# wangsibovictor/fora

Measured on AMD Instinct MI355X. Metric: SSPPR queries/sec at eps=0.5, higher is better.
Workload: dtype u64 fixed-point 2^-62 (f64 at the boundary)

## Files before the change

### fora_amd/csrc/fora_diag.h

```cpp
#pragma once
#include <hip/hip_runtime.h>
#include <stdint.h>

#if defined(FORA_STAMPS) || defined(FORA_STAMPS_SMALL) || defined(FORA_STAMPS_LEVELS) || defined(FORA_PROBE_STORE) || defined(FORA_PROBE_STORE2) || \
    defined(FORA_PROBE_GATHER) || defined(FORA_PROBE_BIN_LOAD) || defined(FORA_PROBE_BIN_RANK) || defined(FORA_PROBE_BIN_STORE) ||              \
    defined(FORA_PROBE_BIN_SYNC) || defined(FORA_PROBE_BIN_LDS) || defined(FORA_PROBE_ACC_LOAD) || defined(FORA_PROBE_ACC_ATOM) ||               \
    defined(FORA_PROBE_ACC_SWEEP) || defined(FORA_DG_FAKE_STEP0) || defined(FORA_DG_FAKE_ALL)
#define FORA_DIAG_BUILD 1
#else
#define FORA_DIAG_BUILD 0
#endif

#ifdef FORA_STAMPS
#define STAMP_DECL long long st_t_ = clock64(); unsigned long long st_a_[8] = {0, 0, 0, 0, 0, 0, 0, 0}; (void)st_a_;
#define STAMP(slot) do { const long long n_ = clock64(); st_a_[(slot) & 7] += (unsigned long long)(n_ - st_t_); st_t_ = n_; } while (0)
#define STAMP_FLUSH(base) do { if (threadIdx.x == 0) for (int i_ = 0; i_ < 8; i_++) if (st_a_[i_]) atomicAdd(&d.stamps[(base) + i_], st_a_[i_]); } while (0)
#define TSTAMP_DECL long long ts_t_ = clock64(); unsigned long long ts_a_[10] = {0, 0, 0, 0, 0, 0, 0, 0, 0, 0}; bool ts_on_ = true; (void)ts_on_;
#ifdef FORA_STAMPS_SMALL
#define TSTAMP(k) do { const long long n_ = clock64(); if (ts_on_) ts_a_[k] += (unsigned long long)(n_ - ts_t_); ts_t_ = n_; } while (0)
#define TSTAMP_GATE(F) do { ts_on_ = (F) <= (uint32_t)(FORA_STAMPS_SMALL) && (F) > 0; if (ts_on_) ts_a_[4]++; } while (0)
#else
#define TSTAMP(k) do { const long long n_ = clock64(); ts_a_[k] += (unsigned long long)(n_ - ts_t_); ts_t_ = n_; } while (0)
#define TSTAMP_GATE(F) do {} while (0)
#endif
// ... 20 lines not shown
namespace fora {
namespace diag {

__device__ __forceinline__ void keep(uint32_t x) { asm volatile("" ::"v"(x)); }
__device__ __forceinline__ void keep(uint64_t x) { asm volatile("" ::"v"(x)); }
__device__ __forceinline__ void keep(const uint4 &x) { asm volatile("" ::"v"(x.x), "v"(x.y), "v"(x.z), "v"(x.w)); }
__device__ __forceinline__ unsigned long long opaque_zero() { unsigned long long z = 0; asm volatile("" : "+v"(z)); return z; }

#if defined(FORA_PROBE_STORE) || defined(FORA_PROBE_STORE2)
constexpr size_t TEAM_MSG_PROBE_WORDS = (size_t)80000000 + (1u << 18);
#else
constexpr size_t TEAM_MSG_PROBE_WORDS = 0;
#endif

template <int EPT>
__device__ __forceinline__ void team_emit_probe(const uint32_t (&word)[EPT], const uint32_t (&dst)[EPT], const uint32_t (&slot)[EPT], uint32_t *mout, uint32_t empty) {
#ifdef FORA_PROBE_STORE2
    {
        const uint32_t base = (uint32_t)__builtin_amdgcn_readfirstlane((int)slot[0]) & ~63u, lane_ = threadIdx.x & 63u;
#pragma unroll
        for (int k = 0; k < EPT; k++)
            mout[(size_t)80000000 + base + k * 4096 + (FORA_PROBE_STORE2 == 1 ? lane_ : (lane_ >> 4) * 1024 + (lane_ & 15u) + 5)] = word[k];
    }
#endif
#ifdef FORA_PROBE_STORE
#pragma unroll
    for (int k = 0; k < EPT; k++)
        if (dst[k] != empty) mout[(size_t)(FORA_PROBE_STORE) + slot[k]] = word[k];
#endif
    (void)word; (void)dst; (void)slot; (void)mout; (void)empty;
}
__device__ __forceinline__ uint64_t team_gather_probe(const uint64_t *tb, uint32_t entry, bool have) {
#ifdef FORA_PROBE_GATHER
    const uint64_t xa = __hip_atomic_load((const unsigned long long *)&tb[have ? (entry ^ 8u) : 0u], __ATOMIC_RELAXED, __HIP_MEMORY_SCOPE_AGENT);
    return xa >> 63;
#else
    (void)tb; (void)entry; (void)have;
    return 0;
#endif
}

__device__ __forceinline__ uint32_t dg_from(uint32_t cur, uint32_t t) {
#if defined(FORA_DG_FAKE_ALL)
    (void)t; return cur & 1023u;
#elif defined(FORA_DG_FAKE_STEP0)
    return t == 0 ? (cur & 1023u) : cur;
#else
    (void)t; return cur;
#endif
}

__device__ __forceinline__ uint4 bin_load_probe(const int32_t *colsrc, const int32_t *col4, const int32_t *col_hub4, const int32_t *col, int64_t quad) {
#if defined(FORA_PROBE_BIN_LOAD) && FORA_PROBE_BIN_LOAD == 2
// ... 98 lines not shown
```

### fora_amd/csrc/fora_hip.hip

```cpp
#include "fora_kernels.h"
#include "fora_team.h"
#include "fora_bwd.h"
#include "../../include/fora_hip.h"

#include <algorithm>
#include <cmath>
#include <cstdio>
#include <cstdlib>
#include <cstring>
#include <string>
#include <vector>

using namespace fora;

struct fora_ctx;
static int build_hub_copy(fora_ctx *c, const int64_t *row_ptr, const int32_t *col);
static int build_quad_copies(fora_ctx *c);
namespace {

struct EvPair {
    hipEvent_t a, b;
    int kind;
};

// ... 29 lines not shown
    int64_t team_hubs = 1024;
    int64_t tail_hubs = 1;
    int64_t team_log = -1;
    int64_t slot_major = -1;
    int64_t acc_group = 0;
    int64_t team_abort_level = 0;
    int64_t team_timeout_ms = 500;
    int64_t team_coop = 0;
    int64_t topk_bk_div = 16;
    int64_t quads = 1;
    int64_t pipeline = 0;
    int64_t profile = 1;
    int64_t grid = 2048;
    int64_t bwd_lds_cap = BWD_CAP_DEFAULT;
    int64_t bwd_chunk = 0;
};
static const struct { const char *name; int64_t Tunables::*field; bool layout; } OPTIONS[] = {
    {"direct", &Tunables::direct, true}, {"force_wide", &Tunables::force_wide, true}, {"pass_bins", &Tunables::pass_bins, true},
    {"no_split", &Tunables::no_split, true}, {"no_compact", &Tunables::no_compact, false}, {"walk_dg", &Tunables::walk_dg, false}, {"dg_hubs", &Tunables::dg_hubs, false}, {"hubs", &Tunables::hubs, true}, {"hubs_wide", &Tunables::hubs_wide, true}, {"hub_min", &Tunables::hub_min, false}, {"bkcap", &Tunables::bkcap, true},
    {"ovcap", &Tunables::ovcap, true}, {"tiny", &Tunables::tiny, false}, {"xb", &Tunables::xb, false}, {"ax", &Tunables::ax, false},
    {"wx", &Tunables::wx, false}, {"tail", &Tunables::tail, false}, {"tail_always", &Tunables::tail_always, false},
    {"select_compact", &Tunables::select_compact, false}, {"pipeline", &Tunables::pipeline, false}, {"team", &Tunables::team, true}, {"team_size", &Tunables::team_size, true}, {"team_tail", &Tunables::team_tail, false}, {"team_xcd", &Tunables::team_xcd, false}, {"team_max", &Tunables::team_max, true}, {"team_hubs", &Tunables::team_hubs, true}, {"team_log", &Tunables::team_log, false}, {"topk_bk_div", &Tunables::topk_bk_div, true}, {"quads", &Tunables::quads, false}, {"team_timeout_ms", &Tunables::team_timeout_ms, false}, {"team_abort_level", &Tunables::team_abort_level, false}, {"acc_group", &Tunables::acc_group, false}, {"slot_major", &Tunables::slot_major, false}, {"team_coop", &Tunables::team_coop, false}, {"tail_hubs", &Tunables::tail_hubs, false}, {"rounds", &Tunables::rounds, false}, {"defer", &Tunables::defer, true}, {"defer_min", &Tunables::defer_min, false}, {"round_div", &Tunables::round_div, false},
    {"profile", &Tunables::profile, false}, {"grid", &Tunables::grid, false},
    {"bwd_lds_cap", &Tunables::bwd_lds_cap, false}, {"bwd_chunk", &Tunables::bwd_chunk, false},
};
static bool schedule_option(const char *name) {
    return !strcmp(name, "rounds") || !strcmp(name, "round_div") || !strcmp(name, "defer") || !strcmp(name, "defer_min");
}
static Tunables tunables_from_env() {
    Tunables t;
    for (const auto &o : OPTIONS) {
        if (schedule_option(o.name)) continue;
        std::string env = "FORA_HIP_";
        for (const char *p = o.name; *p; p++) env += (char)toupper((unsigned char)*p);
        if (const char *e = getenv(env.c_str())) if (*e) t.*(o.field) = atoll(e);
    }
    return t;
}

struct fora_ctx {
    int device = 0;
    Tunables opt_;
    hipStream_t stream = nullptr;
    std::string err;
    hipDeviceProp_t prop{};

    int32_t n = 0;
// ... 18 lines not shown
    uint64_t *d_hubsum = nullptr;
    uint32_t *d_dg_perm = nullptr, *d_dg_inv = nullptr, *d_dg_colp = nullptr, *d_dg_rec = nullptr, *d_dg_invb = nullptr;
    uint8_t *d_dg_T = nullptr;
    WalkDG dg{};
    uint32_t *d_colt = nullptr, *d_team_off = nullptr, *d_team_n2l = nullptr, *d_team_l2n = nullptr;
    uint32_t *d_team_hubtgt = nullptr;
    uint32_t team_H = 0, team_hubs_opt = 0;
    uint16_t *d_team_rlog_id = nullptr; uint64_t *d_team_rlog_val = nullptr; uint32_t team_rlog_cap = 0;
    uint64_t *d_team_rowl = nullptr, *d_team_rsvl = nullptr;
    uint16_t *d_team_deg16 = nullptr;
    uint32_t *d_team_rowq = nullptr;
    uint32_t team_T = 0, team_R = 0, team_force = 0;
    bool team_checked = false, team_wanted = false;
    double dangling_frac = 0;
    uint64_t team_cap = 0;
    uint32_t *d_team_msg = nullptr;
    uint64_t *d_team_inct = nullptr;
    unsigned long long *d_team_cnt = nullptr;
    uint32_t *d_team_ctl = nullptr;
    uint32_t team_n = 0;
    bool team_dirty = false;
    bool hub_for_team = false;
    bool team_timeout_seen = false;
    int team_suspend = 0;
    uint64_t team_fallbacks = 0;
    int team_fit = -1;
    bool team_coop_ok = false;
    bool team_coop_failed = false;

    bool have_params = false;
    double alpha = 0.2, epsilon = 0.5, rmax_scale = 1.0, rmax = 0, omega = 0;
// ... 381 lines not shown
               c->wit_cap >= pe.wits && c->bk_cap == pe.bk_cap && c->sub == pe.sub;
    };
    {
        int need = c->batch_req > 0 ? c->batch_req : std::min(want_slots > 0 ? want_slots : 1024, 1024);
        if (c->batch_req == 0 && c->B > 0 && c->B_memcap > 0) need = std::min(need, c->B_memcap);
        if (keepable(need)) { const WsPlan pe = plan_workspace(c, omega_hint, c->B); return ensure_row_split(c, pe.nbins, pe.pbins); }
    }
    int B = c->batch_req > 0 ? c->batch_req : 0;
    if (B == 0) {
        free_workspace(c);
        size_t fr = 0, tot = 0;
        HIPCHK(c, hipMemGetInfo(&fr, &tot));
        uint64_t budget = (uint64_t)(fr * (c->opt_.pipeline == 1 ? 0.4 : 0.75));
        if (c->team_T) {
            const uint64_t T = c->team_T, nt = std::max<uint64_t>(1, (uint64_t)c->prop.multiProcessorCount * TEAM_WGS_PER_CU / T);
            const uint64_t team_bytes = nt * (2 * c->team_cap * 4 + 3 * T * (c->team_R + 64 + c->team_H) * 8 + T * (10ull << 17) + 2 * T * T * 8);
            budget -= std::min<uint64_t>(budget / 2, team_bytes);
        }
        B = (int)std::min<uint64_t>(1024, std::max<uint64_t>(1, budget / p.per_slot));
    }
    B = std::max(1, B);
    const int memcap = B;
    if (want_slots > 0 && c->batch_req == 0) B = std::min(B, std::max(want_slots, 1));
    p = plan_workspace(c, omega_hint, B);
    const uint64_t scratch = (uint64_t)B * p.scratch;
    free_workspace(c);
    const uint64_t slab = (uint64_t)B * n;
    HIPCHK(c, hipMalloc(&c->d_residue, slab * 8));
    HIPCHK(c, hipMalloc(&c->d_ppr, slab * 8));
    if (p.binned) {
        HIPCHK(c, hipMalloc(&c->d_fl[0], slab * 4));
// ... 12 lines not shown
        HIPCHK(c, hipMalloc(&c->d_bk_count, (size_t)B * p.pbins * p.sub * 4));
        HIPCHK(c, hipHostMalloc(&c->h_flc, (size_t)FLC_RING * B * 4 * CSTRIDE));
        c->dbm_words = (uint32_t)((uint64_t)p.nbins << (bin_shift(c) - 6));
        HIPCHK(c, hipMalloc(&c->d_dbm, 2 * (size_t)B * c->dbm_words * 8));
        HIPCHK(c, hipMalloc(&c->d_dflag, 2 * (size_t)B * p.nbins * 4));
        if (c->opt_.defer > 0) HIPCHK(c, hipMalloc(&c->d_dl, 2 * slab * 4));
        if (c->hubs && c->hub_shift == bin_shift(c)) HIPCHK(c, hipMalloc(&c->d_hubsum, (size_t)B * p.sub * c->hubs * 8));
        if (c->team_T) {
            const uint32_t T = c->team_T;
            uint32_t nteams = std::max<uint32_t>(1, (uint32_t)c->prop.multiProcessorCount * TEAM_WGS_PER_CU / T);
            if (c->opt_.team_max > 0) nteams = std::min<uint32_t>(nteams, (uint32_t)c->opt_.team_max);
            size_t fr = 0, tot = 0;
            HIPCHK(c, hipMemGetInfo(&fr, &tot));
            c->team_rlog_cap = 1u << 17;
            auto per_team_bytes = [&](uint32_t logcap) {
                return 2 * c->team_cap * 4 + 3 * (uint64_t)T * (c->team_R + 64 + c->team_H) * 8 + (uint64_t)T * logcap * 10 + 2 * (uint64_t)T * T * 8;
            };
            while (c->team_rlog_cap > 1024 && per_team_bytes(c->team_rlog_cap) > fr / 4) c->team_rlog_cap /= 2;
            const uint64_t per_team = per_team_bytes(c->team_rlog_cap);
            nteams = (uint32_t)std::max<uint64_t>(1, std::min<uint64_t>(nteams, (uint64_t)(fr / 2) / std::max<uint64_t>(1, per_team)));
            HIPCHK(c, hipMalloc(&c->d_team_msg, (size_t)nteams * 2 * c->team_cap * 4 + 64 + diag::TEAM_MSG_PROBE_WORDS * 4));
            HIPCHK(c, hipMalloc(&c->d_team_inct, (size_t)nteams * 2 * T * (c->team_R + 64 + c->team_H) * 8));
            HIPCHK(c, hipMalloc(&c->d_team_rsvl, (size_t)nteams * T * c->team_R * 8));
            HIPCHK(c, hipMemset(c->d_team_rsvl, 0, (size_t)nteams * T * c->team_R * 8));
            HIPCHK(c, hipMalloc(&c->d_team_rlog_id, (size_t)nteams * T * c->team_rlog_cap * 2));
            HIPCHK(c, hipMalloc(&c->d_team_rlog_val, (size_t)nteams * T * c->team_rlog_cap * 8));
            HIPCHK(c, hipMalloc(&c->d_team_cnt, (size_t)nteams * 2 * T * T * 8));
            HIPCHK(c, hipMalloc(&c->d_team_ctl, (64 + (size_t)nteams * 5 * 16 * 2 + (size_t)nteams * ((size_t)B + 2)) * 4));
            c->team_n = nteams;
            if (int rf = team_fits(c)) return rf;
        }
    } else {
        HIPCHK(c, hipMalloc(&c->d_wl[0], slab * 8));
        HIPCHK(c, hipMalloc(&c->d_wl[1], slab * 8));
    }
    HIPCHK(c, hipMalloc(&c->d_scratch, scratch));
// ... 321 lines not shown
    a.residue = d.residue; a.ppr = d.ppr; a.fl0 = d.fl[0]; a.fl_count0 = d.fl_count[0]; a.inc_tab0 = d.inc_tab[0];
    a.segq_cap = d.segq_cap; a.qs = d.qs; a.err = d.err; a.afix = d.afix; a.t1 = d.t1;
    a.T = T; a.R = c->team_R; a.nteams = nteams;
    a.colt = c->d_colt; a.rowq = c->d_team_rowq; a.n2l = c->d_team_n2l; a.l2n = c->d_team_l2n; a.deg16 = c->d_team_deg16; a.rowl = c->d_team_rowl; a.rsvl = c->d_team_rsvl; a.rlog_id = c->d_team_rlog_id; a.rlog_val = c->d_team_rlog_val; a.rlog_cap = c->opt_.team_log == 0 ? 0u : c->opt_.team_log > 0 ? std::min<uint32_t>((uint32_t)c->opt_.team_log, c->team_rlog_cap) : c->team_rlog_cap; a.H = c->team_H; a.hubtgt = c->d_team_hubtgt; a.off = c->d_team_off; a.msg = c->d_team_msg; a.inct = c->d_team_inct; a.cntw = c->d_team_cnt;
    a.ctl = c->d_team_ctl;
    a.sync = (unsigned long long *)(c->d_team_ctl + 64);
    a.slot_seq = c->d_team_ctl + 64 + (size_t)nteams * 5 * 16 * 2;
    const int64_t tail_auto = 4096;
    a.tail_max = (uint32_t)std::min<int64_t>(std::max<int64_t>(c->opt_.team_tail < 0 ? tail_auto : c->opt_.team_tail, 0), 0x7FFFFFFF);
    if (c->opt_.tail == 0) a.tail_max = 0;
    a.tail_always = c->opt_.tail_always == 1 ? 1u : 0u;
    const uint32_t grid = nteams * T;
    a.xcd = (c->opt_.team_xcd >= 1 && grid % 8 == 0 && (grid / 8) % T == 0) ? (uint32_t)c->opt_.team_xcd : 0u;
    a.stamps = c->d_stamps;
    a.abort_level = (uint32_t)std::min<int64_t>(std::max<int64_t>(c->opt_.team_abort_level, 0), 1 << 20);
    a.timeout_ticks = (uint64_t)std::min<int64_t>(std::max<int64_t>(c->opt_.team_timeout_ms, 0), 60000) * 100000ull;
    const size_t lds = ((size_t)a.R + 1 + a.H) * 8;
    if (c->team_dirty) { HIPCHK(c, hipMemsetAsync(c->d_team_rsvl, 0, (size_t)nteams * T * c->team_R * 8, c->stream)); c->team_dirty = false; }
    HIPCHK(c, hipMemsetAsync(c->d_team_ctl, 0, (64 + (size_t)nteams * 5 * 16 * 2) * 4, c->stream));
    HIPCHK(c, hipMemsetAsync(c->d_team_cnt, 0, (size_t)nteams * 2 * T * T * 8, c->stream));
    HIPCHK(c, hipMemsetAsync(a.slot_seq, 0xFF, (size_t)nteams * ((size_t)d.nq + 2) * 4, c->stream));
    int h = ev_begin(c, 10);
    bool launched = false;
    if (c->team_coop_ok && !c->team_coop_failed) {
        void *args[] = {(void *)&a};
        const hipError_t le = hipLaunchCooperativeKernel((const void *)k_push_team, dim3(grid), dim3(TEAM_THREADS), args, (unsigned)lds, c->stream);
        if (le == hipSuccess) launched = true;
        else { (void)hipGetLastError(); c->team_coop_failed = true; }
    }
    if (!launched) hipLaunchKernelGGL(k_push_team, dim3(grid), dim3(TEAM_THREADS), lds, c->stream, a);
// ... 829 lines not shown
int fora_hip_get_batch(fora_ctx *c) { return c ? c->B : FORA_E_ARG; }

int fora_hip_set_option(fora_ctx *c, const char *name, int64_t value) {
    if (!c || !name) return FORA_E_ARG;
    if (!strcmp(name, "reset")) {
        (void)hipSetDevice(c->device);
        free_workspace(c);
        if (c->twin) free_workspace(c->twin);
        c->opt_ = tunables_from_env();
        c->team_suspend = 0;
        c->profiling = c->opt_.profile != 0;
        c->grid_blocks = c->opt_.grid > 0 ? (int)c->opt_.grid : 2048;
        if (c->twin) { c->twin->opt_ = c->opt_; c->twin->grid_blocks = c->grid_blocks; }
        return FORA_OK;
    }
    if (!TEST_PATHS && schedule_option(name) && value != (strcmp(name, "rounds") ? (strcmp(name, "round_div") ? 0 : 4) : 1))
        return fail(c, FORA_E_ARG, std::string("option ") + name + ": the schedule experiments are not compiled into this library (build with -DFORA_TEST_PATHS=1: libfora_hip_test.so)");
    for (const auto &o : OPTIONS)
        if (!strcmp(name, o.name)) {
            if (c->opt_.*(o.field) == value) return FORA_OK;
            c->opt_.*(o.field) = value;
            if (o.layout) { (void)hipSetDevice(c->device); free_workspace(c); if (c->twin) free_workspace(c->twin); }
            if (!strcmp(name, "profile")) c->profiling = value != 0;
            if (!strcmp(name, "grid")) { c->grid_blocks = value > 0 ? (int)value : 2048; if (c->twin) c->twin->grid_blocks = c->grid_blocks; }
            return FORA_OK;
        }
    return fail(c, FORA_E_ARG, std::string("unknown option ") + name);
}

int fora_hip_get_option(fora_ctx *c, const char *name, int64_t *value) {
    if (!name || !value) return FORA_E_ARG;
// ... 1139 lines not shown
```

### fora_amd/csrc/fora_team.h

```cpp
#pragma once
#include "fora_kernels.h"

namespace fora {

constexpr int TEAM_MAX = 32;
constexpr int TEAM_LBITS = 15;
#ifndef FORA_TEAM_THREADS
#define FORA_TEAM_THREADS 1024
#endif
constexpr int TEAM_THREADS = FORA_TEAM_THREADS;
#ifndef FORA_TEAM_WGS_PER_CU
#define FORA_TEAM_WGS_PER_CU (FORA_TEAM_THREADS == 1024 ? 1 : 2)
#endif
constexpr int TEAM_WGS_PER_CU = FORA_TEAM_WGS_PER_CU;
constexpr int TEAM_NW = TEAM_THREADS / 64;
constexpr uint32_t TEAM_R_CAP = TEAM_WGS_PER_CU == 1 ? 15296 : 7680;
constexpr int TEAM_NIT = (TEAM_R_CAP + TEAM_THREADS - 1) / TEAM_THREADS;
#ifndef FORA_TEAM_EPT
#define FORA_TEAM_EPT 4
#endif
#ifndef FORA_TEAM_CU
#define FORA_TEAM_CU 4
#endif
#ifndef FORA_TEAM_MPL
#define FORA_TEAM_MPL 2
#endif
#ifndef FORA_TEAM_DRAW
#define FORA_TEAM_DRAW 4
#endif
constexpr int TEAM_EPT = FORA_TEAM_EPT;
constexpr int TEAM_CHUNK = 64 * TEAM_EPT;
constexpr uint32_t TEAM_LMASK = (1u << TEAM_LBITS) - 1u;
constexpr uint32_t TEAM_EMPTY = 0xFFFFFFFFu;
constexpr uint32_t ERR_TEAM_TIMEOUT = 16, ERR_TEAM_CAP = 32;

struct TeamDev {
    int32_t n, nq;
    const uint64_t *rowinfo;
    const int64_t *row_ptr;
    const uint32_t *deg;
    const int32_t *src;
    uint64_t *residue, *ppr;
    uint32_t *fl0, *fl_count0;
    uint64_t *inc_tab0;
    uint64_t segq_cap;
    QState *qs;
    uint32_t *err;
    uint64_t afix, t1;
    uint32_t T, R, nteams;
    const uint32_t *colt;
    const uint32_t *rowq;
    const uint32_t *n2l;
    const uint32_t *l2n;
    const uint16_t *deg16;
    const uint64_t *rowl;
    uint64_t *rsvl;
    uint16_t *rlog_id;
    uint64_t *rlog_val;
    uint32_t rlog_cap;
    uint32_t H;
    const uint32_t *hubtgt;
    const uint32_t *off;
    uint32_t *msg;
    uint64_t *inct;
    unsigned long long *cntw;
    unsigned long long *sync;
    uint32_t *slot_seq;
    uint32_t *ctl;
    uint32_t tail_max;
    uint32_t tail_always;
    uint32_t xcd;
    unsigned long long *stamps;
    uint64_t timeout_ticks;
    uint32_t abort_level;
};

typedef const __attribute__((address_space(4))) TeamDev *TeamArgs;
__device__ __forceinline__ TeamArgs team_args() {
    TeamArgs p = (TeamArgs)__builtin_amdgcn_kernarg_segment_ptr();
    asm volatile("" : "+s"(p));
    return p;
}

__device__ __forceinline__ uint32_t rank_below(unsigned long long mk) {
    return __builtin_amdgcn_mbcnt_hi((uint32_t)(mk >> 32), __builtin_amdgcn_mbcnt_lo((uint32_t)mk, 0u));
}
__device__ __forceinline__ int fresh(int x) { asm volatile("" : "+v"(x)); return x; }
__device__ __forceinline__ uint32_t fresh_s(uint32_t x) { asm volatile("" : "+s"(x)); return x; }

// ... 26 lines not shown


#ifndef FORA_TEAM_HEAVY
#define FORA_TEAM_HEAVY 1024
#endif
constexpr uint32_t TEAM_HEAVY = FORA_TEAM_HEAVY;
#ifndef FORA_TEAM_NHEAVY
#define FORA_TEAM_NHEAVY 128
#endif
#ifndef FORA_TEAM_MAXGROUPS
#define FORA_TEAM_MAXGROUPS 256
#endif
constexpr int TEAM_NHEAVY = FORA_TEAM_NHEAVY;
constexpr int TEAM_MAXGROUPS = FORA_TEAM_MAXGROUPS;

__device__ __forceinline__ void team_emit(const uint32_t (&word)[TEAM_EPT], const uint32_t (&dst)[TEAM_EPT], uint32_t *s_fill, uint32_t *mout) {
    uint32_t slot[TEAM_EPT];
#pragma unroll
    for (int k = 0; k < TEAM_EPT; k++) {
        slot[k] = 0;
        if (dst[k] != TEAM_EMPTY) slot[k] = atomicAdd(&s_fill[dst[k]], 1u);
    }
#pragma unroll
    for (int k = 0; k < TEAM_EPT; k++)
        if (dst[k] != TEAM_EMPTY) mout[slot[k]] = word[k];
    diag::team_emit_probe(word, dst, slot, mout, TEAM_EMPTY);
}

__global__ void __launch_bounds__(TEAM_THREADS, TEAM_THREADS * TEAM_WGS_PER_CU / 256) k_push_team(const TeamDev kernarg_only) {
    extern __shared__ uint64_t res[];
    __shared__ uint16_t w_list[TEAM_NW][128];
// ... 107 lines not shown
            src_spare = src_word == TEAM_EMPTY;
            src_local = src_spare ? R : (src_word & TEAM_LMASK);
        }
        uint64_t acc_res = 0, acc_pops = 0, acc_relax = 0;
        uint32_t peak = 0, nlev = 0;
        uint32_t logbase = 0;
        bool final_round = false;
        if (fresh(tid0) == 0) s_rsvovf = 0;

        TSTAMP_LEVEL_DECL
        for (uint32_t L = 0;; L++) {
            const int tid = fresh(tid0), lane = tid & 63, wid = __builtin_amdgcn_readfirstlane(tid >> 6);
            if (L > 0) {
                const TeamArgs a = team_args();
                const uint32_t par = (g - 1) & 1u;
                const uint32_t *min_ = a->msg + ((uint64_t)team * 2 + par) * cap_total;
                const uint64_t *tin = a->inct + ((uint64_t)team * 2 + par) * T * tstride;
                const uint32_t tagp = g & 0xFFFFFFu;
                const unsigned long long *cwin = a->cntw + ((uint64_t)team * 2 + par) * T * T + (uint64_t)me * T;
                const unsigned long long full = T >= 64 ? ~0ull : (1ull << T) - 1ull;
                unsigned long long donemask = 0;
                uint32_t fsum = 0, spins = 0;
                uint64_t w_t0 = 0;
                while (donemask != full) {
                unsigned long long wv = 0;
                if ((uint32_t)lane < T) wv = __hip_atomic_load(&cwin[lane], __ATOMIC_RELAXED, __HIP_MEMORY_SCOPE_AGENT);
                const unsigned long long ready = __ballot((uint32_t)lane < T && (uint32_t)(wv >> 40) == tagp) & ~donemask;
                if (!ready) {
                    TSTAMP_SLEEP(8, 2, 40);
                    if ((++spins & 255u) == 0) {
                        const TeamArgs ar = team_args();
// ... 3 lines not shown
                        bool stop = __hip_atomic_load(&ctl[32], __ATOMIC_RELAXED, __HIP_MEMORY_SCOPE_AGENT) != 0;
                        if (!stop && now - w_t0 > ar->timeout_ticks) {
                            __hip_atomic_store(&ctl[32], 1u, __ATOMIC_RELAXED, __HIP_MEMORY_SCOPE_AGENT);
                            if (lane == 0) atomicOr(ar->err, ERR_TEAM_TIMEOUT);
                            stop = true;
                        }
                        if (stop) { if (lane == 0) s_abort = 1u; break; }
                    }
                    continue;
                }
                if (!same_xcd) { __builtin_amdgcn_fence(__ATOMIC_ACQUIRE, "agent"); asm volatile("s_waitcnt vmcnt(0)" ::: "memory"); }
                donemask |= ready;
                const bool mine = (ready >> lane) & 1ull;
                const uint32_t c = mine ? (uint32_t)wv & 0xFFFFFFu : 0u;
                fsum += mine ? (uint32_t)(wv >> 24) & 0xFFFFu : 0u;
                constexpr int MPL = FORA_TEAM_MPL, SEGSH = MPL == 4 ? 8 : 7;
                constexpr int CU = MPL == 4 ? (FORA_TEAM_CU + 1) / 2 : FORA_TEAM_CU;
                const uint32_t ns = (c + (1u << SEGSH) - 1u) >> SEGSH;
                const uint32_t r0 = ((uint32_t)wid + 2u * TEAM_NW - (uint32_t)lane % TEAM_NW) % TEAM_NW;
                const uint32_t kmine = ns > r0 ? (ns - r0 + TEAM_NW - 1) / TEAM_NW : 0u;
                uint32_t nmine;
                const uint32_t pmine = wave_excl_scan(kmine, nmine);
                for (uint32_t i0 = 0; i0 < nmine; i0 += CU) {
                    uint32_t mw[CU][MPL];
                    uint4 mq[CU];
                    uint32_t srcm[CU], left[CU];
                    const uint32_t *mp[CU];
#pragma unroll
                    for (int k = 0; k < CU; k++) {
                        const bool have = i0 + k < nmine;
                        const uint32_t ic = have ? i0 + k : 0u;
                        const uint32_t sidx = (uint32_t)__popcll(__ballot(pmine <= ic)) - 1u;
                        const uint32_t j = (uint32_t)__builtin_amdgcn_readlane((int)r0, (int)sidx) + (ic - (uint32_t)__builtin_amdgcn_readlane((int)pmine, (int)sidx)) * TEAM_NW;
                        const uint32_t n_s = (uint32_t)__builtin_amdgcn_readlane((int)c, (int)sidx);
                        const uint32_t idx = (j << SEGSH) + (uint32_t)MPL * lane;
                        left[k] = (have && idx < n_s) ? n_s - idx : 0u;
                        srcm[k] = sidx;
                        mp[k] = min_ + (uint64_t)(uint32_t)__builtin_amdgcn_readlane((int)coffv, (int)sidx) + (left[k] ? idx : 0u);
                        if (MPL != 4) {
                            const unsigned long long mm = __hip_atomic_load((const unsigned long long *)mp[k], __ATOMIC_RELAXED, __HIP_MEMORY_SCOPE_AGENT);
                            mw[k][0] = (uint32_t)mm; mw[k][1] = (uint32_t)(mm >> 32);
                        }
                    }
                    if (MPL == 4) {
                        static_assert(MPL != 4 || CU <= 2, "one asm statement per trip");
                        if (CU == 1) asm volatile("global_load_dwordx4 %0, %1, off sc1\n\ts_waitcnt vmcnt(0)" : "=&v"(mq[0]) : "v"(mp[0]) : "memory");
                        else asm volatile("global_load_dwordx4 %0, %2, off sc1\n\tglobal_load_dwordx4 %1, %3, off sc1\n\ts_waitcnt vmcnt(0)"
                                          : "=&v"(mq[0]), "=&v"(mq[CU - 1]) : "v"(mp[0]), "v"(mp[CU - 1]) : "memory");
#pragma unroll
                        for (int k = 0; k < CU; k++) { mw[k][0] = mq[k].x; mw[k][1] = mq[k].y; mw[k][MPL - 2] = mq[k].z; mw[k][MPL - 1] = mq[k].w; }
                    }
                    uint64_t vv[CU][MPL];
#pragma unroll
                    for (int k = 0; k < CU; k++) {
                        const uint64_t *tb = tin + (uint64_t)srcm[k] * tstride;
#pragma unroll
                        for (int u = 0; u < MPL; u++)
                            vv[k][u] = __hip_atomic_load((const unsigned long long *)&tb[left[k] > (uint32_t)u ? (mw[k][u] >> TEAM_LBITS) : 0u], __ATOMIC_RELAXED, __HIP_MEMORY_SCOPE_AGENT);
                    }
#pragma unroll
                    for (int k = 0; k < CU; k++)
#pragma unroll
                        for (int u = 0; u < MPL; u++)
                            vv[k][u] += diag::team_gather_probe(tin + (uint64_t)srcm[k] * tstride, mw[k][u] >> TEAM_LBITS, left[k] > (uint32_t)u);
#pragma unroll
                    for (int k = 0; k < CU; k++)
#pragma unroll
                        for (int u = 0; u < MPL; u++)
                            if (left[k] > (uint32_t)u && vv[k][u]) atomicAdd((unsigned long long *)&res[mw[k][u] & TEAM_LMASK], (unsigned long long)vv[k][u]);
                }
                }
                if (wid == 0) {
                    const uint32_t fs = wave_incl_scan_add(fsum);
                    if (lane == 63) s_F = fs;
                }
                __syncthreads();
                TSTAMP_GATE(s_F);
                TSTAMP(0);
                const TeamArgs af = team_args();
                bool quit = s_abort != 0;
                if (af->abort_level && L == af->abort_level) {
                    if (tid == 0) { __hip_atomic_store(&af->ctl[32], 1u, __ATOMIC_RELAXED, __HIP_MEMORY_SCOPE_AGENT); atomicOr(af->err, ERR_TEAM_TIMEOUT); }
                    quit = true;
                }
// ... 149 lines not shown
                    for (int it = 0; it < TEAM_NIT; it++) {
                        if ((uint32_t)it * TEAM_THREADS + (uint32_t)wid * 64u < R) {
                            const uint32_t l = it * TEAM_THREADS + tid;
                            uint64_t rs = res[l];
                            if (ovf) { const uint64_t o = rsvl[l]; if (o) { rs += o; rsvl[l] = 0; } }
                            if (rs) { ppr[lv[it]] = rs; res[l] = 0; }
                        }
                    }
                }
                TSTAMP(6);
                break;
            }
            uint64_t my_dang = 0;
            {
                const TeamArgs a = team_args();
                uint32_t *mout = a->msg + ((uint64_t)team * 2 + (g & 1u)) * cap_total;
                uint64_t *tout = a->inct + (((uint64_t)team * 2 + (g & 1u)) * T + me) * tstride;
                const uint64_t *rowl = a->rowl + (uint64_t)me * R;
                const uint32_t rlog_cap = a->rlog_cap;
                uint16_t *rlog_id = a->rlog_id + ((uint64_t)team * T + me) * rlog_cap;
                uint64_t *rlog_val = a->rlog_val + ((uint64_t)team * T + me) * rlog_cap;
                const uint64_t afix = a->afix;
                const uint32_t *colt = a->colt;
                uint16_t *list = w_list[wid];
                uint64_t *winc = w_inc[wid];
                uint8_t *mark = w_mark[wid];
                uint32_t npend = 0, gcur = 0, gend = 0;
                bool drained = false;
                constexpr uint32_t bsz = 64;
                if (L == 0) { drained = true; if (me == src_owner && wid == 0) { if (lane == 0) list[0] = (uint16_t)src_local; npend = 1; } }
                for (;;) {
                    while (npend < bsz) {
// ... 32 lines not shown
                        const uint64_t rr = res[l];
                        res[l] = 0;
                        uint32_t deg = spare ? src_deg : (uint32_t)(rw >> 19) & 8191u;
                        if (!spare && deg == 8191u) deg = team_args()->deg[(uint32_t)rw & 0x7FFFFu];
                        uint64_t rsv_add, dang;
                        const uint64_t inc = pop_value(afix, rr, deg, rsv_add, dang);
                        if (logi < rlog_cap) { rlog_val[logi] = direct ? 0ull : rsv_add; rlog_id[logi] = direct ? (uint16_t)0 : (uint16_t)l; }
                        if (direct && rsv_add) {
                            const TeamArgs ar = team_args();
                            if (spare) ar->ppr[slab + src] = rsv_old + rsv_add;
                            else { (ar->rsvl + ((uint64_t)team * T + me) * R)[l] = rsv_old + rsv_add; s_rsvovf = 1u; }
                        }
                        acc_res += rsv_add; my_dang += dang; acc_pops++; acc_relax += deg;
                        ebeg = spare ? srcq : (uint32_t)(rw >> 32);
                        cnt = inc ? deg : 0u;
                        if (cnt) tout[ebase + lane] = inc;
                        winc[lane] = inc;
                        if (cnt > TEAM_HEAVY) {
                            const uint32_t hi = atomicAdd(&s_nheavy, 1u);
                            if (hi < (uint32_t)TEAM_NHEAVY) {
                                h_ent[hi] = ebase + lane; h_ebeg[hi] = ebeg; h_inc[hi] = inc;
                                h_cstart[hi] = atomicAdd(&s_hchunks, (cnt + TEAM_CHUNK - 1) / TEAM_CHUNK);
                                __atomic_store_n(&h_deg[hi], cnt, __ATOMIC_RELEASE);
                                cnt = 0;
                            }
                        }
                    }
                    if (npend > 64) {
                        const uint16_t keep = list[64 + (lane < 63 ? lane : 63)];
                        __builtin_amdgcn_wave_barrier();
                        if ((uint32_t)lane < npend - 64) list[lane] = keep;
// ... 11 lines not shown
                        if (lane < 16) ((uint32_t *)mark)[lane] = 0;
                        __builtin_amdgcn_wave_barrier();
                        if (qn && pre - cb < 64u) mark[pre - cb] = (uint8_t)(lane + 1);
                        __builtin_amdgcn_wave_barrier();
                        const uint32_t mk = mark[lane];
                        const uint32_t x = wave_incl_scan_max(mk);
                        const uint32_t lastx = (uint32_t)__builtin_amdgcn_readlane((int)x, 63);
                        const uint32_t row1 = x ? x : carry;
                        if (lastx) carry = lastx;
                        const uint32_t si = row1 ? row1 - 1u : 0u;
                        const uint32_t q = cb + lane;
                        const uint32_t rb = (uint32_t)__shfl((int)rowbase, (int)si);
                        uint4 w4 = colt4[q < total ? rb + q : 0u];
                        if (q >= total) w4 = make_uint4(TEAM_EMPTY, TEAM_EMPTY, TEAM_EMPTY, TEAM_EMPTY);
                        const uint32_t w[TEAM_EPT] = {w4.x, w4.y, w4.z, w4.w};
                        const uint32_t entw = (ebase + si) << TEAM_LBITS;
                        uint32_t word[TEAM_EPT], dst[TEAM_EPT];
#pragma unroll
                        for (int k = 0; k < TEAM_EPT; k++) {
                            dst[k] = w[k] == TEAM_EMPTY ? TEAM_EMPTY : w[k] >> TEAM_LBITS;
                            word[k] = (w[k] & TEAM_LMASK) | entw;
                            if (w[k] != TEAM_EMPTY && (w[k] & 0x80000000u)) {
                                atomicAdd(&s_hub[w[k] & 0x7FFFFFFFu], (unsigned long long)winc[si]);
                                dst[k] = TEAM_EMPTY;
                            }
                        }
                        team_emit(word, dst, s_fill, mout);
                    }
                    TSTAMP(3);
                }
            }
            TSTAMP(2);
            my_dang = wave_sum(my_dang);
            if (lane == 0 && my_dang) atomicAdd(&s_dang, (unsigned long long)my_dang);
            {
                if (lane == 0) atomicAdd(&s_wdone, 1u);
                for (;;) {
                    uint32_t k = TEAM_EMPTY, fin = 0;
                    if (lane == 0) {
                        const uint32_t nx = __atomic_load_n(&s_hnext, __ATOMIC_RELAXED), tot = __atomic_load_n(&s_hchunks, __ATOMIC_RELAXED);
                        if (nx < tot) { if (atomicCAS(&s_hnext, nx, nx + 1u) == nx) k = nx; }
                        else if (__atomic_load_n(&s_wdone, __ATOMIC_RELAXED) == (uint32_t)TEAM_NW && nx >= __atomic_load_n(&s_hchunks, __ATOMIC_RELAXED)) fin = 1;
                    }
                    k = (uint32_t)__builtin_amdgcn_readfirstlane((int)k);
                    fin = (uint32_t)__builtin_amdgcn_readfirstlane((int)fin);
                    if (fin) break;
                    if (k == TEAM_EMPTY) { TSTAMP_SLEEP(9, 1, 30); continue; }
                    const TeamArgs a = team_args();
                    uint32_t *mout = a->msg + ((uint64_t)team * 2 + (g & 1u)) * cap_total;
                    const uint32_t *colt = a->colt;
                    uint32_t eb = 0, dgh = 0, ent = 0, c0 = 0;
                    uint64_t hinc = 0;
                    for (bool found = false; !found;) {
                        const uint32_t nh = min(__atomic_load_n(&s_nheavy, __ATOMIC_RELAXED), (uint32_t)TEAM_NHEAVY);
                        for (uint32_t hb = 0; hb < nh && !found; hb += 64) {
                            const uint32_t h = hb + lane;
                            const uint32_t dg = h < nh ? __atomic_load_n(&h_deg[h], __ATOMIC_ACQUIRE) : 0u;
                            const uint32_t cs = dg ? h_cstart[h] : 0u;
                            const unsigned long long hit = __ballot(dg && k >= cs && k < cs + (dg + TEAM_CHUNK - 1) / TEAM_CHUNK);
                            if (hit) {
                                const uint32_t hs = hb + (uint32_t)__ffsll((long long)hit) - 1u;
                                eb = h_ebeg[hs]; dgh = h_deg[hs]; ent = h_ent[hs] << TEAM_LBITS; hinc = h_inc[hs]; c0 = (k - h_cstart[hs]) * TEAM_CHUNK;
                                found = true;
                            }
                        }
                    }
                    uint32_t word[TEAM_EPT], dst[TEAM_EPT];
                    {
                        const uint32_t q = (c0 >> 2) + lane;
                        uint4 w4 = make_uint4(TEAM_EMPTY, TEAM_EMPTY, TEAM_EMPTY, TEAM_EMPTY);
                        if (q < ((dgh + 3u) >> 2)) w4 = ((const uint4 *)colt)[(uint64_t)eb + q];
                        const uint32_t w[TEAM_EPT] = {w4.x, w4.y, w4.z, w4.w};
#pragma unroll
                        for (int kk = 0; kk < TEAM_EPT; kk++) {
                            dst[kk] = TEAM_EMPTY; word[kk] = 0;
                            if (w[kk] != TEAM_EMPTY) {
                                if (w[kk] & 0x80000000u) atomicAdd(&s_hub[w[kk] & 0x7FFFFFFFu], (unsigned long long)hinc);
                                else { dst[kk] = w[kk] >> TEAM_LBITS; word[kk] = (w[kk] & TEAM_LMASK) | ent; }
                            }
                        }
                    }
                    team_emit(word, dst, s_fill, mout);
                }
            }
            TSTAMP(6);
            __syncthreads();
            TSTAMP(7);
            {
                const TeamArgs a = team_args();
                uint32_t *mout = a->msg + ((uint64_t)team * 2 + (g & 1u)) * cap_total;
                uint64_t *tout = a->inct + (((uint64_t)team * 2 + (g & 1u)) * T + me) * tstride;
                if (tid == 0 && s_dang) {
                    const uint32_t ent = s_ncross, pos = atomicAdd(&s_fill[src_owner], 1u);
                    tout[ent] = s_dang;
                    mout[pos] = src_local | (ent << TEAM_LBITS);
                }
                if ((uint32_t)tid < H) {
                    const uint32_t *hubtgt = a->hubtgt;
                    for (uint32_t h = tid; h < H; h += TEAM_THREADS) {
                        const unsigned long long hv = s_hub[h];
                        if (hv) {
                            s_hub[h] = 0;
                            const uint32_t tg = h < (uint32_t)TEAM_THREADS ? hub_tg0 : hubtgt[h], ent = s_ncross + 1 + atomicAdd(&s_hubent, 1u);
                            tout[ent] = hv;
                            mout[atomicAdd(&s_fill[tg >> TEAM_LBITS], 1u)] = (tg & TEAM_LMASK) | (ent << TEAM_LBITS);
                        }
                    }
                }
                asm volatile("s_waitcnt vmcnt(0)" ::: "memory");
                __syncthreads();
                const uint32_t tag = (g + 1u) & 0xFFFFFFu;
                if (!same_xcd) {
                    if (tid == 0) { __builtin_amdgcn_fence(__ATOMIC_RELEASE, "agent"); asm volatile("s_waitcnt vmcnt(0)" ::: "memory"); }
                    __syncthreads();
                }
                if ((uint32_t)tid < T) {
                    unsigned long long *cw = team_args()->cntw + ((uint64_t)team * 2 + (g & 1u)) * T * T;
                    __hip_atomic_store(&cw[(uint32_t)tid * T + me], (unsigned long long)(s_fill[tid] - s_moff[tid]) | ((unsigned long long)s_ncross << 24) | ((unsigned long long)tag << 40),
                                       __ATOMIC_RELAXED, __HIP_MEMORY_SCOPE_AGENT);
                }
// ... 31 lines not shown
```

Baseline: 6775.

## Inline increment values into 64-bit team messages, escaping only large values

```diff
diff --git a/fora_amd/csrc/fora_diag.h b/fora_amd/csrc/fora_diag.h
--- a/fora_amd/csrc/fora_diag.h
+++ b/fora_amd/csrc/fora_diag.h
@@ -5,7 +5,7 @@
 #if defined(FORA_STAMPS) || defined(FORA_STAMPS_SMALL) || defined(FORA_STAMPS_LEVELS) || defined(FORA_PROBE_STORE) || defined(FORA_PROBE_STORE2) || \
     defined(FORA_PROBE_GATHER) || defined(FORA_PROBE_BIN_LOAD) || defined(FORA_PROBE_BIN_RANK) || defined(FORA_PROBE_BIN_STORE) ||              \
     defined(FORA_PROBE_BIN_SYNC) || defined(FORA_PROBE_BIN_LDS) || defined(FORA_PROBE_ACC_LOAD) || defined(FORA_PROBE_ACC_ATOM) ||               \
-    defined(FORA_PROBE_ACC_SWEEP) || defined(FORA_DG_FAKE_STEP0) || defined(FORA_DG_FAKE_ALL)
+    defined(FORA_PROBE_ACC_SWEEP) || defined(FORA_DG_FAKE_STEP0) || defined(FORA_DG_FAKE_ALL) || defined(FORA_COUNT_ESCAPES)
 #define FORA_DIAG_BUILD 1
 #else
 #define FORA_DIAG_BUILD 0
@@ -58,7 +58,7 @@
 #endif
 
 template <int EPT>
-__device__ __forceinline__ void team_emit_probe(const uint32_t (&word)[EPT], const uint32_t (&dst)[EPT], const uint32_t (&slot)[EPT], uint32_t *mout, uint32_t empty) {
+__device__ __forceinline__ void team_emit_probe(const uint64_t (&word)[EPT], const uint32_t (&dst)[EPT], const uint32_t (&slot)[EPT], uint64_t *mout, uint32_t empty) {
 #ifdef FORA_PROBE_STORE2
     {
         const uint32_t base = (uint32_t)__builtin_amdgcn_readfirstlane((int)slot[0]) & ~63u, lane_ = threadIdx.x & 63u;
@@ -81,6 +81,24 @@
 #else
     (void)tb; (void)entry; (void)have;
     return 0;
+#endif
+}
+
+template <int CU>
+__device__ __forceinline__ void team_esc_count(const uint32_t (&left)[CU], const uint64_t (&mw)[CU], uint64_t esc, unsigned long long *stamps) {
+#ifdef FORA_COUNT_ESCAPES
+    uint32_t nm = 0, ne = 0;
+#pragma unroll
+    for (int k = 0; k < CU; k++) {
+        nm += (uint32_t)__popcll(__ballot(left[k] != 0));
+        ne += (uint32_t)__popcll(__ballot(left[k] != 0 && (mw[k] & esc)));
+    }
+    if ((threadIdx.x & 63u) == 0) {
+        if (nm) atomicAdd(&stamps[12], (unsigned long long)nm);
+        if (ne) atomicAdd(&stamps[13], (unsigned long long)ne);
+    }
+#else
+    (void)left; (void)mw; (void)esc; (void)stamps;
 #endif
 }
 
diff --git a/fora_amd/csrc/fora_hip.hip b/fora_amd/csrc/fora_hip.hip
--- a/fora_amd/csrc/fora_hip.hip
+++ b/fora_amd/csrc/fora_hip.hip
@@ -67,6 +67,7 @@
     int64_t grid = 2048;
     int64_t bwd_lds_cap = BWD_CAP_DEFAULT;
     int64_t bwd_chunk = 0;
+    int64_t team_escape = 0;
 };
 static const struct { const char *name; int64_t Tunables::*field; bool layout; } OPTIONS[] = {
     {"direct", &Tunables::direct, true}, {"force_wide", &Tunables::force_wide, true}, {"pass_bins", &Tunables::pass_bins, true},
@@ -76,14 +77,16 @@
     {"select_compact", &Tunables::select_compact, false}, {"pipeline", &Tunables::pipeline, false}, {"team", &Tunables::team, true}, {"team_size", &Tunables::team_size, true}, {"team_tail", &Tunables::team_tail, false}, {"team_xcd", &Tunables::team_xcd, false}, {"team_max", &Tunables::team_max, true}, {"team_hubs", &Tunables::team_hubs, true}, {"team_log", &Tunables::team_log, false}, {"topk_bk_div", &Tunables::topk_bk_div, true}, {"quads", &Tunables::quads, false}, {"team_timeout_ms", &Tunables::team_timeout_ms, false}, {"team_abort_level", &Tunables::team_abort_level, false}, {"acc_group", &Tunables::acc_group, false}, {"slot_major", &Tunables::slot_major, false}, {"team_coop", &Tunables::team_coop, false}, {"tail_hubs", &Tunables::tail_hubs, false}, {"rounds", &Tunables::rounds, false}, {"defer", &Tunables::defer, true}, {"defer_min", &Tunables::defer_min, false}, {"round_div", &Tunables::round_div, false},
     {"profile", &Tunables::profile, false}, {"grid", &Tunables::grid, false},
     {"bwd_lds_cap", &Tunables::bwd_lds_cap, false}, {"bwd_chunk", &Tunables::bwd_chunk, false},
+    {"team_escape", &Tunables::team_escape, false},
 };
 static bool schedule_option(const char *name) {
     return !strcmp(name, "rounds") || !strcmp(name, "round_div") || !strcmp(name, "defer") || !strcmp(name, "defer_min");
 }
+static bool test_option(const char *name) { return schedule_option(name) || !strcmp(name, "team_escape"); }
 static Tunables tunables_from_env() {
     Tunables t;
     for (const auto &o : OPTIONS) {
-        if (schedule_option(o.name)) continue;
+        if (test_option(o.name)) continue;
         std::string env = "FORA_HIP_";
         for (const char *p = o.name; *p; p++) env += (char)toupper((unsigned char)*p);
         if (const char *e = getenv(env.c_str())) if (*e) t.*(o.field) = atoll(e);
@@ -132,7 +135,7 @@
     bool team_checked = false, team_wanted = false;
     double dangling_frac = 0;
     uint64_t team_cap = 0;
-    uint32_t *d_team_msg = nullptr;
+    uint64_t *d_team_msg = nullptr;
     uint64_t *d_team_inct = nullptr;
     unsigned long long *d_team_cnt = nullptr;
     uint32_t *d_team_ctl = nullptr;
@@ -544,7 +547,7 @@
         uint64_t budget = (uint64_t)(fr * (c->opt_.pipeline == 1 ? 0.4 : 0.75));
         if (c->team_T) {
             const uint64_t T = c->team_T, nt = std::max<uint64_t>(1, (uint64_t)c->prop.multiProcessorCount * TEAM_WGS_PER_CU / T);
-            const uint64_t team_bytes = nt * (2 * c->team_cap * 4 + 3 * T * (c->team_R + 64 + c->team_H) * 8 + T * (10ull << 17) + 2 * T * T * 8);
+            const uint64_t team_bytes = nt * (2 * c->team_cap * 8 + 3 * T * (c->team_R + 64 + c->team_H) * 8 + T * (10ull << 17) + 2 * T * T * 8);
             budget -= std::min<uint64_t>(budget / 2, team_bytes);
         }
         B = (int)std::min<uint64_t>(1024, std::max<uint64_t>(1, budget / p.per_slot));
@@ -587,12 +590,12 @@
             HIPCHK(c, hipMemGetInfo(&fr, &tot));
             c->team_rlog_cap = 1u << 17;
             auto per_team_bytes = [&](uint32_t logcap) {
-                return 2 * c->team_cap * 4 + 3 * (uint64_t)T * (c->team_R + 64 + c->team_H) * 8 + (uint64_t)T * logcap * 10 + 2 * (uint64_t)T * T * 8;
+                return 2 * c->team_cap * 8 + 3 * (uint64_t)T * (c->team_R + 64 + c->team_H) * 8 + (uint64_t)T * logcap * 10 + 2 * (uint64_t)T * T * 8;
             };
             while (c->team_rlog_cap > 1024 && per_team_bytes(c->team_rlog_cap) > fr / 4) c->team_rlog_cap /= 2;
             const uint64_t per_team = per_team_bytes(c->team_rlog_cap);
             nteams = (uint32_t)std::max<uint64_t>(1, std::min<uint64_t>(nteams, (uint64_t)(fr / 2) / std::max<uint64_t>(1, per_team)));
-            HIPCHK(c, hipMalloc(&c->d_team_msg, (size_t)nteams * 2 * c->team_cap * 4 + 64 + diag::TEAM_MSG_PROBE_WORDS * 4));
+            HIPCHK(c, hipMalloc(&c->d_team_msg, (size_t)nteams * 2 * c->team_cap * 8 + 128 + diag::TEAM_MSG_PROBE_WORDS * 8));
             HIPCHK(c, hipMalloc(&c->d_team_inct, (size_t)nteams * 2 * T * (c->team_R + 64 + c->team_H) * 8));
             HIPCHK(c, hipMalloc(&c->d_team_rsvl, (size_t)nteams * T * c->team_R * 8));
             HIPCHK(c, hipMemset(c->d_team_rsvl, 0, (size_t)nteams * T * c->team_R * 8));
@@ -944,6 +947,7 @@
     a.xcd = (c->opt_.team_xcd >= 1 && grid % 8 == 0 && (grid / 8) % T == 0) ? (uint32_t)c->opt_.team_xcd : 0u;
     a.stamps = c->d_stamps;
     a.abort_level = (uint32_t)std::min<int64_t>(std::max<int64_t>(c->opt_.team_abort_level, 0), 1 << 20);
+    a.esc_all = TEST_PATHS && c->opt_.team_escape != 0 ? 1u : 0u;
     a.timeout_ticks = (uint64_t)std::min<int64_t>(std::max<int64_t>(c->opt_.team_timeout_ms, 0), 60000) * 100000ull;
     const size_t lds = ((size_t)a.R + 1 + a.H) * 8;
     if (c->team_dirty) { HIPCHK(c, hipMemsetAsync(c->d_team_rsvl, 0, (size_t)nteams * T * c->team_R * 8, c->stream)); c->team_dirty = false; }
@@ -1803,7 +1807,7 @@
         if (c->twin) { c->twin->opt_ = c->opt_; c->twin->grid_blocks = c->grid_blocks; }
         return FORA_OK;
     }
-    if (!TEST_PATHS && schedule_option(name) && value != (strcmp(name, "rounds") ? (strcmp(name, "round_div") ? 0 : 4) : 1))
+    if (!TEST_PATHS && test_option(name) && value != (strcmp(name, "rounds") ? (strcmp(name, "round_div") ? 0 : 4) : 1))
         return fail(c, FORA_E_ARG, std::string("option ") + name + ": the schedule experiments are not compiled into this library (build with -DFORA_TEST_PATHS=1: libfora_hip_test.so)");
     for (const auto &o : OPTIONS)
         if (!strcmp(name, o.name)) {
diff --git a/fora_amd/csrc/fora_team.h b/fora_amd/csrc/fora_team.h
--- a/fora_amd/csrc/fora_team.h
+++ b/fora_amd/csrc/fora_team.h
@@ -22,9 +22,6 @@
 #ifndef FORA_TEAM_CU
 #define FORA_TEAM_CU 4
 #endif
-#ifndef FORA_TEAM_MPL
-#define FORA_TEAM_MPL 2
-#endif
 #ifndef FORA_TEAM_DRAW
 #define FORA_TEAM_DRAW 4
 #endif
@@ -33,6 +30,14 @@
 constexpr uint32_t TEAM_LMASK = (1u << TEAM_LBITS) - 1u;
 constexpr uint32_t TEAM_EMPTY = 0xFFFFFFFFu;
 constexpr uint32_t ERR_TEAM_TIMEOUT = 16, ERR_TEAM_CAP = 32;
+constexpr int TEAM_VSHIFT = TEAM_LBITS + 1;
+constexpr uint64_t TEAM_ESC = 1ull << TEAM_LBITS;
+constexpr uint64_t TEAM_INLINE_LIM = 1ull << (64 - TEAM_VSHIFT);
+
+__device__ __forceinline__ bool team_escapes(uint64_t inc, bool esc_all) { return inc >= TEAM_INLINE_LIM || esc_all; }
+__device__ __forceinline__ uint64_t team_val(uint64_t inc, uint32_t ent, bool esc_all) {
+    return team_escapes(inc, esc_all) ? (TEAM_ESC | (uint64_t)ent << TEAM_VSHIFT) : inc << TEAM_VSHIFT;
+}
 
 struct TeamDev {
     int32_t n, nq;
@@ -61,7 +66,7 @@
     uint32_t H;
     const uint32_t *hubtgt;
     const uint32_t *off;
-    uint32_t *msg;
+    uint64_t *msg;
     uint64_t *inct;
     unsigned long long *cntw;
     unsigned long long *sync;
@@ -73,6 +78,7 @@
     unsigned long long *stamps;
     uint64_t timeout_ticks;
     uint32_t abort_level;
+    uint32_t esc_all;
 };
 
 typedef const __attribute__((address_space(4))) TeamDev *TeamArgs;
@@ -129,7 +135,7 @@
 constexpr int TEAM_NHEAVY = FORA_TEAM_NHEAVY;
 constexpr int TEAM_MAXGROUPS = FORA_TEAM_MAXGROUPS;
 
-__device__ __forceinline__ void team_emit(const uint32_t (&word)[TEAM_EPT], const uint32_t (&dst)[TEAM_EPT], uint32_t *s_fill, uint32_t *mout) {
+__device__ __forceinline__ void team_emit(const uint64_t (&word)[TEAM_EPT], const uint32_t (&dst)[TEAM_EPT], uint32_t *s_fill, uint64_t *mout) {
     uint32_t slot[TEAM_EPT];
 #pragma unroll
     for (int k = 0; k < TEAM_EPT; k++) {
@@ -267,7 +273,7 @@
             if (L > 0) {
                 const TeamArgs a = team_args();
                 const uint32_t par = (g - 1) & 1u;
-                const uint32_t *min_ = a->msg + ((uint64_t)team * 2 + par) * cap_total;
+                const uint64_t *min_ = a->msg + ((uint64_t)team * 2 + par) * cap_total;
                 const uint64_t *tin = a->inct + ((uint64_t)team * 2 + par) * T * tstride;
                 const uint32_t tagp = g & 0xFFFFFFu;
                 const unsigned long long *cwin = a->cntw + ((uint64_t)team * 2 + par) * T * T + (uint64_t)me * T;
@@ -301,18 +307,15 @@
                 const bool mine = (ready >> lane) & 1ull;
                 const uint32_t c = mine ? (uint32_t)wv & 0xFFFFFFu : 0u;
                 fsum += mine ? (uint32_t)(wv >> 24) & 0xFFFFu : 0u;
-                constexpr int MPL = FORA_TEAM_MPL, SEGSH = MPL == 4 ? 8 : 7;
-                constexpr int CU = MPL == 4 ? (FORA_TEAM_CU + 1) / 2 : FORA_TEAM_CU;
+                constexpr int SEGSH = 6, CU = FORA_TEAM_CU;
                 const uint32_t ns = (c + (1u << SEGSH) - 1u) >> SEGSH;
                 const uint32_t r0 = ((uint32_t)wid + 2u * TEAM_NW - (uint32_t)lane % TEAM_NW) % TEAM_NW;
                 const uint32_t kmine = ns > r0 ? (ns - r0 + TEAM_NW - 1) / TEAM_NW : 0u;
                 uint32_t nmine;
                 const uint32_t pmine = wave_excl_scan(kmine, nmine);
                 for (uint32_t i0 = 0; i0 < nmine; i0 += CU) {
-                    uint32_t mw[CU][MPL];
-                    uint4 mq[CU];
+                    uint64_t mw[CU];
                     uint32_t srcm[CU], left[CU];
-                    const uint32_t *mp[CU];
 #pragma unroll
                     for (int k = 0; k < CU; k++) {
                         const bool have = i0 + k < nmine;
@@ -320,41 +323,37 @@
                         const uint32_t sidx = (uint32_t)__popcll(__ballot(pmine <= ic)) - 1u;
                         const uint32_t j = (uint32_t)__builtin_amdgcn_readlane((int)r0, (int)sidx) + (ic - (uint32_t)__builtin_amdgcn_readlane((int)pmine, (int)sidx)) * TEAM_NW;
                         const uint32_t n_s = (uint32_t)__builtin_amdgcn_readlane((int)c, (int)sidx);
-                        const uint32_t idx = (j << SEGSH) + (uint32_t)MPL * lane;
+                        const uint32_t idx = (j << SEGSH) + (uint32_t)lane;
                         left[k] = (have && idx < n_s) ? n_s - idx : 0u;
                         srcm[k] = sidx;
-                        mp[k] = min_ + (uint64_t)(uint32_t)__builtin_amdgcn_readlane((int)coffv, (int)sidx) + (left[k] ? idx : 0u);
-                        if (MPL != 4) {
-                            const unsigned long long mm = __hip_atomic_load((const unsigned long long *)mp[k], __ATOMIC_RELAXED, __HIP_MEMORY_SCOPE_AGENT);
-                            mw[k][0] = (uint32_t)mm; mw[k][1] = (uint32_t)(mm >> 32);
-                        }
-                    }
-                    if (MPL == 4) {
-                        static_assert(MPL != 4 || CU <= 2, "one asm statement per trip");
-                        if (CU == 1) asm volatile("global_load_dwordx4 %0, %1, off sc1\n\ts_waitcnt vmcnt(0)" : "=&v"(mq[0]) : "v"(mp[0]) : "memory");
-                        else asm volatile("global_load_dwordx4 %0, %2, off sc1\n\tglobal_load_dwordx4 %1, %3, off sc1\n\ts_waitcnt vmcnt(0)"
-                                          : "=&v"(mq[0]), "=&v"(mq[CU - 1]) : "v"(mp[0]), "v"(mp[CU - 1]) : "memory");
-#pragma unroll
-                        for (int k = 0; k < CU; k++) { mw[k][0] = mq[k].x; mw[k][1] = mq[k].y; mw[k][MPL - 2] = mq[k].z; mw[k][MPL - 1] = mq[k].w; }
-                    }
-                    uint64_t vv[CU][MPL];
+                        const uint64_t *mp = min_ + (uint64_t)(uint32_t)__builtin_amdgcn_readlane((int)coffv, (int)sidx) + (left[k] ? idx : 0u);
+                        mw[k] = __hip_atomic_load((const unsigned long long *)mp, __ATOMIC_RELAXED, __HIP_MEMORY_SCOPE_AGENT);
+                    }
+                    uint64_t vv[CU];
+                    bool esc = false;
 #pragma unroll
                     for (int k = 0; k < CU; k++) {
-                        const uint64_t *tb = tin + (uint64_t)srcm[k] * tstride;
-#pragma unroll
-                        for (int u = 0; u < MPL; u++)
-                            vv[k][u] = __hip_atomic_load((const unsigned long long *)&tb[left[k] > (uint32_t)u ? (mw[k][u] >> TEAM_LBITS) : 0u], __ATOMIC_RELAXED, __HIP_MEMORY_SCOPE_AGENT);
-                    }
+                        vv[k] = mw[k] >> TEAM_VSHIFT;
+                        esc |= left[k] && (mw[k] & TEAM_ESC);
+                    }
+                    if (__ballot(esc)) {
+                        uint64_t gv[CU];
+#pragma unroll
+                        for (int k = 0; k < CU; k++) {
+                            const bool e = left[k] && (mw[k] & TEAM_ESC);
+                            gv[k] = __hip_atomic_load((const unsigned long long *)(tin + (uint64_t)srcm[k] * tstride + (e ? (uint32_t)vv[k] : 0u)), __ATOMIC_RELAXED, __HIP_MEMORY_SCOPE_AGENT);
+                        }
+#pragma unroll
+                        for (int k = 0; k < CU; k++)
+                            if (left[k] && (mw[k] & TEAM_ESC)) vv[k] = gv[k];
+                    }
+                    diag::team_esc_count(left, mw, TEAM_ESC, a->stamps);
 #pragma unroll
                     for (int k = 0; k < CU; k++)
-#pragma unroll
-                        for (int u = 0; u < MPL; u++)
-                            vv[k][u] += diag::team_gather_probe(tin + (uint64_t)srcm[k] * tstride, mw[k][u] >> TEAM_LBITS, left[k] > (uint32_t)u);
+                        vv[k] += diag::team_gather_probe(tin + (uint64_t)srcm[k] * tstride, (uint32_t)mw[k] & TEAM_LMASK, left[k] != 0);
 #pragma unroll
                     for (int k = 0; k < CU; k++)
-#pragma unroll
-                        for (int u = 0; u < MPL; u++)
-                            if (left[k] > (uint32_t)u && vv[k][u]) atomicAdd((unsigned long long *)&res[mw[k][u] & TEAM_LMASK], (unsigned long long)vv[k][u]);
+                        if (left[k] && vv[k]) atomicAdd((unsigned long long *)&res[mw[k] & TEAM_LMASK], (unsigned long long)vv[k]);
                 }
                 }
                 if (wid == 0) {
@@ -534,8 +533,9 @@
             uint64_t my_dang = 0;
             {
                 const TeamArgs a = team_args();
-                uint32_t *mout = a->msg + ((uint64_t)team * 2 + (g & 1u)) * cap_total;
+                uint64_t *mout = a->msg + ((uint64_t)team * 2 + (g & 1u)) * cap_total;
                 uint64_t *tout = a->inct + (((uint64_t)team * 2 + (g & 1u)) * T + me) * tstride;
+                const bool esc_all = TEST_PATHS && a->esc_all != 0;
                 const uint64_t *rowl = a->rowl + (uint64_t)me * R;
                 const uint32_t rlog_cap = a->rlog_cap;
                 uint16_t *rlog_id = a->rlog_id + ((uint64_t)team * T + me) * rlog_cap;
@@ -598,7 +598,7 @@
                         acc_res += rsv_add; my_dang += dang; acc_pops++; acc_relax += deg;
                         ebeg = spare ? srcq : (uint32_t)(rw >> 32);
                         cnt = inc ? deg : 0u;
-                        if (cnt) tout[ebase + lane] = inc;
+                        if (cnt && team_escapes(inc, esc_all)) tout[ebase + lane] = inc;
                         winc[lane] = inc;
                         if (cnt > TEAM_HEAVY) {
                             const uint32_t hi = atomicAdd(&s_nheavy, 1u);
@@ -640,14 +640,16 @@
                         uint4 w4 = colt4[q < total ? rb + q : 0u];
                         if (q >= total) w4 = make_uint4(TEAM_EMPTY, TEAM_EMPTY, TEAM_EMPTY, TEAM_EMPTY);
                         const uint32_t w[TEAM_EPT] = {w4.x, w4.y, w4.z, w4.w};
-                        const uint32_t entw = (ebase + si) << TEAM_LBITS;
-                        uint32_t word[TEAM_EPT], dst[TEAM_EPT];
+                        const uint64_t rinc = winc[si];
+                        const uint64_t hiw = team_val(rinc, ebase + si, esc_all);
+                        uint64_t word[TEAM_EPT];
+                        uint32_t dst[TEAM_EPT];
 #pragma unroll
                         for (int k = 0; k < TEAM_EPT; k++) {
                             dst[k] = w[k] == TEAM_EMPTY ? TEAM_EMPTY : w[k] >> TEAM_LBITS;
-                            word[k] = (w[k] & TEAM_LMASK) | entw;
+                            word[k] = (uint64_t)(w[k] & TEAM_LMASK) | hiw;
                             if (w[k] != TEAM_EMPTY && (w[k] & 0x80000000u)) {
-                                atomicAdd(&s_hub[w[k] & 0x7FFFFFFFu], (unsigned long long)winc[si]);
+                                atomicAdd(&s_hub[w[k] & 0x7FFFFFFFu], (unsigned long long)rinc);
                                 dst[k] = TEAM_EMPTY;
                             }
                         }
@@ -673,7 +675,7 @@
                     if (fin) break;
                     if (k == TEAM_EMPTY) { TSTAMP_SLEEP(9, 1, 30); continue; }
                     const TeamArgs a = team_args();
-                    uint32_t *mout = a->msg + ((uint64_t)team * 2 + (g & 1u)) * cap_total;
+                    uint64_t *mout = a->msg + ((uint64_t)team * 2 + (g & 1u)) * cap_total;
                     const uint32_t *colt = a->colt;
                     uint32_t eb = 0, dgh = 0, ent = 0, c0 = 0;
                     uint64_t hinc = 0;
@@ -686,12 +688,14 @@
                             const unsigned long long hit = __ballot(dg && k >= cs && k < cs + (dg + TEAM_CHUNK - 1) / TEAM_CHUNK);
                             if (hit) {
                                 const uint32_t hs = hb + (uint32_t)__ffsll((long long)hit) - 1u;
-                                eb = h_ebeg[hs]; dgh = h_deg[hs]; ent = h_ent[hs] << TEAM_LBITS; hinc = h_inc[hs]; c0 = (k - h_cstart[hs]) * TEAM_CHUNK;
+                                eb = h_ebeg[hs]; dgh = h_deg[hs]; ent = h_ent[hs]; hinc = h_inc[hs]; c0 = (k - h_cstart[hs]) * TEAM_CHUNK;
                                 found = true;
                             }
                         }
                     }
-                    uint32_t word[TEAM_EPT], dst[TEAM_EPT];
+                    const uint64_t hiw = team_val(hinc, ent, TEST_PATHS && a->esc_all != 0);
+                    uint64_t word[TEAM_EPT];
+                    uint32_t dst[TEAM_EPT];
                     {
                         const uint32_t q = (c0 >> 2) + lane;
                         uint4 w4 = make_uint4(TEAM_EMPTY, TEAM_EMPTY, TEAM_EMPTY, TEAM_EMPTY);
@@ -702,7 +706,7 @@
                             dst[kk] = TEAM_EMPTY; word[kk] = 0;
                             if (w[kk] != TEAM_EMPTY) {
                                 if (w[kk] & 0x80000000u) atomicAdd(&s_hub[w[kk] & 0x7FFFFFFFu], (unsigned long long)hinc);
-                                else { dst[kk] = w[kk] >> TEAM_LBITS; word[kk] = (w[kk] & TEAM_LMASK) | ent; }
+                                else { dst[kk] = w[kk] >> TEAM_LBITS; word[kk] = (uint64_t)(w[kk] & TEAM_LMASK) | hiw; }
                             }
                         }
                     }
@@ -714,12 +718,14 @@
             TSTAMP(7);
             {
                 const TeamArgs a = team_args();
-                uint32_t *mout = a->msg + ((uint64_t)team * 2 + (g & 1u)) * cap_total;
+                uint64_t *mout = a->msg + ((uint64_t)team * 2 + (g & 1u)) * cap_total;
                 uint64_t *tout = a->inct + (((uint64_t)team * 2 + (g & 1u)) * T + me) * tstride;
+                const bool esc_all = TEST_PATHS && a->esc_all != 0;
                 if (tid == 0 && s_dang) {
                     const uint32_t ent = s_ncross, pos = atomicAdd(&s_fill[src_owner], 1u);
-                    tout[ent] = s_dang;
-                    mout[pos] = src_local | (ent << TEAM_LBITS);
+                    const uint64_t dv = s_dang;
+                    if (team_escapes(dv, esc_all)) tout[ent] = dv;
+                    mout[pos] = (uint64_t)src_local | team_val(dv, ent, esc_all);
                 }
                 if ((uint32_t)tid < H) {
                     const uint32_t *hubtgt = a->hubtgt;
@@ -727,9 +733,10 @@
                         const unsigned long long hv = s_hub[h];
                         if (hv) {
                             s_hub[h] = 0;
-                            const uint32_t tg = h < (uint32_t)TEAM_THREADS ? hub_tg0 : hubtgt[h], ent = s_ncross + 1 + atomicAdd(&s_hubent, 1u);
-                            tout[ent] = hv;
-                            mout[atomicAdd(&s_fill[tg >> TEAM_LBITS], 1u)] = (tg & TEAM_LMASK) | (ent << TEAM_LBITS);
+                            const bool e = team_escapes(hv, esc_all);
+                            const uint32_t tg = h < (uint32_t)TEAM_THREADS ? hub_tg0 : hubtgt[h], ent = e ? s_ncross + 1 + atomicAdd(&s_hubent, 1u) : 0u;
+                            if (e) tout[ent] = hv;
+                            mout[atomicAdd(&s_fill[tg >> TEAM_LBITS], 1u)] = (uint64_t)(tg & TEAM_LMASK) | team_val(hv, ent, esc_all);
                         }
                     }
                 }
```

Result: no change. 6832, median of 6 (+0.8%).
